# MoseleyBioinformaticsLab/ICIKendallTau

Measured on AMD Instinct MI355X. Metric: column-pairs/s (+ full-matrix wall time) at 10k feat x 1k samp, higher is better.
Workload: dtype int32 rank/popcount counting + f64 epilogue

## Files before the change

### icikendalltau_amd/csrc/icikt_capi.cpp

```cpp
#include <hip/hip_runtime.h>

#include <algorithm>
#include <chrono>
#include <cstdio>
#include <cstring>
#include <functional>
#include <new>
#include <string>
#include <vector>

#include "icikt.h"
#include "icikt_device.h"
#include "icikt_host.h"

using icikt::ColStats;
using icikt::PairRaw;
using icikt::PrepView;

static_assert(ICIKT_CNT_FIELDS == icikt::ICIKT_CNT_FIELDS_, "counts record layout");
static_assert(ICIKT_PERSPECTIVE_LOCAL == icikt::ICIKT_PERSPECTIVE_LOCAL_, "perspective code");

namespace {

int flush_timer(icikt_ctx* c, int k) {
// ... 578 lines not shown
  pv.sort_keys = c->sort_keys.p; pv.sort_idx = c->sort_idx.p;
  pv.tgroups = c->tgroups.p;
  pv.tprog = c->tprog.p;
  pv.srow = c->srow.p;
  pv.smask = c->smask.p;
  if (pv.wide) {
    pv.order32 = c->wide32.p;
    pv.q32 = pv.order32 + S * (size_t)pv.n_pad;
    pv.lo32 = pv.q32 + S * (size_t)pv.n_pad;
    pv.hi32 = pv.lo32 + S * (size_t)pv.n_pad;
    pv.k0_bits = c->k0_bits.p;
  }
  c->pv = pv;
  c->alloc_cols = (int64_t)S;
  return ICIKT_SUCCESS;
}

int mask_alloc(icikt_ctx* c, int64_t n_feat, int64_t n_samp) {
  c->prepared = false;
  c->raw_valid = false;
  PrepView pv{};
  pv.n = (int)n_feat;
  pv.n_pad = std::max(64, (int)((n_feat + 63) / 64 * 64));
  pv.W = (int)((n_feat + 63) / 64);
  pv.Wp = pv.W + 1;
  pv.n_samp = (int)n_samp;
  pv.mstride = pv.Wp;
  HIPCHK(c, c->meta.reserve((size_t)std::max<int64_t>(n_samp, 1) * (size_t)pv.mstride));
  pv.meta = c->meta.p;
  c->pv = pv;
  return ICIKT_SUCCESS;
}

int prepare_launch(icikt_ctx* c, const double* dX, int64_t ld, int64_t col_begin, int64_t col_end, hipStream_t stream) {
  const PrepView& pv = c->pv;
  if (!stream) stream = c->stream;
  c->raw_valid = false;
  c->tied_state = -1;
  c->ntg_hint = -1;
  c->group_hint = 0;
  if (col_end > col_begin)
    HIPCHK(c, hipMemsetAsync(c->meta.p + (size_t)col_begin * pv.mstride, 0,
                             (size_t)(col_end - col_begin) * pv.mstride * sizeof(unsigned long long), stream));
  if (pv.n > 0) {
    const int64_t chunk = std::max(1, c->sort_chunk);
    for (int64_t c0 = col_begin; c0 < col_end; c0 += chunk) {
      const int nc = (int)std::min<int64_t>(chunk, col_end - c0);
      const int small_shape = (c->k0_shape == 1 || (c->k0_shape < 0 && c->k0_small)) ? 1 : 0;
      HIPCHK(c, icikt::launch_k0(pv, dX, ld, (int)c0, nc, c->k0_mask, c->k0_keep, small_shape, stream));
    }
  }
  return ICIKT_SUCCESS;
}

}
}

using icikt::host::prepare_alloc;
using icikt::host::prepare_launch;

static int prepare_impl(icikt_ctx* c, const double* dX, int64_t n_feat, int64_t n_samp, int64_t ld,
                        int64_t col_begin, int64_t col_end, int64_t alloc_cols, uint32_t flags) {
  if (!c) return ICIKT_E_INVALID;
  int rc = check_shape(c, "prepare", n_feat, n_samp, ld);
  if (rc) return rc;
  if (n_samp > 0 && n_feat > 0 && !dX) return fail(c, ICIKT_E_INVALID, "prepare: null matrix");
  rc = check_col_range(c, n_samp, col_begin, col_end, alloc_cols, n_feat);
  if (rc) return rc;
  rc = use_device(c);
  if (rc) return rc;
  rc = prepare_alloc(c, n_feat, n_samp, alloc_cols, col_end - col_begin);
  if (rc) return rc;
  rc = timer_begin(c, ICIKT_K_PREPARE, flags);
  if (rc) return rc;
  rc = prepare_launch(c, dX, ld, col_begin, col_end);
  if (rc) return rc;
  rc = timer_end(c, ICIKT_K_PREPARE, flags);
  if (rc) return rc;
  c->prepared = true;
  return ICIKT_SUCCESS;
}

// ... 836 lines not shown
extern "C" {

int icikt_debug_set_plan(icikt_ctx* c, const char* spec) {
  if (!c) return ICIKT_E_INVALID;
  icikt_ctx::PlanOverride ov;
  int pipe = -1, k0 = -1;
  std::string sp = spec ? spec : "";
  size_t pos = 0;
  while (pos < sp.size()) {
    size_t end = sp.find(',', pos);
    if (end == std::string::npos) end = sp.size();
    const std::string item = sp.substr(pos, end - pos);
    pos = end + 1;
    if (item.empty()) continue;
    const size_t eq = item.find('=');
    if (eq == std::string::npos) return fail(c, ICIKT_E_INVALID, "debug_set_plan: expected key=value, got '" + item + "'");
    const std::string key = item.substr(0, eq), val = item.substr(eq + 1);
    if (val.empty()) continue;
    if (key == "np") ov.np = atoi(val.c_str());
    else if (key == "pend") ov.pend = (val[0] == 'g') ? 1 : 0;
    else if (key == "wpb") ov.wpb = atoi(val.c_str());
    else if (key == "half") ov.half = (val[0] == '1') ? 1 : 0;
    else if (key == "hyb") ov.hyb = (val[0] == '1') ? 1 : 0;
    else if (key == "tgmax") { ov.has_tgmax = true; ov.tgmax = atoi(val.c_str()); }
    else if (key == "list") ov.list = atoi(val.c_str());
    else if (key == "solo") ov.solo = atoi(val.c_str());
    else if (key == "split") ov.split = atoi(val.c_str());
    else if (key == "merge") ov.merge = atoi(val.c_str());
    else if (key == "waves") ov.waves = atoi(val.c_str());
    else if (key == "verbose") ov.verbose = (val[0] == '1');
    else if (key == "gridmult") ov.grid_mult = atoi(val.c_str());
    else if (key == "gridcap") ov.grid_cap = atoi(val.c_str());
    else if (key == "pipe") pipe = (val[0] == '1') ? 1 : 0;
    else if (key == "k0") k0 = (val[0] == '1') ? 1 : 0;
    else if (key == "tkblock") ov.tkblock = atoll(val.c_str());
    else if (key == "medlds") {
      ov.medlds = atoi(val.c_str());
      if (ov.medlds < 0 || ov.medlds > icikt::MEDIAN_STAGE_MAX)
        return fail(c, ICIKT_E_INVALID, "debug_set_plan: medlds must be in 0 .. 4096 keys");
    }
    else if (key == "qbatch") {
      ov.qbatch = atoi(val.c_str());
      if (ov.qbatch < 1 || ov.qbatch > icikt::QUANT_BATCH_MAX)
        return fail(c, ICIKT_E_INVALID, "debug_set_plan: qbatch must be in 1 .. 32 targets");
    }
    else if (key == "padjtile") {
      ov.padjtile = atoll(val.c_str());
      if (ov.padjtile < 1 || ov.padjtile > (1ll << 30))
        return fail(c, ICIKT_E_INVALID, "debug_set_plan: padjtile must be in 1 .. 2^30 keys");
    }
    else if (key == "anoperms") {
      ov.anoperms = atoll(val.c_str());
      if (ov.anoperms < 1 || ov.anoperms > icikt::ANO_PERMS_MAX)
        return fail(c, ICIKT_E_INVALID, "debug_set_plan: anoperms must be in 1 .. 2^20 labellings");
    }
    else if (key == "anostrip") {
      ov.anostrip = atoi(val.c_str());
      if (ov.anostrip < icikt::ANO_STRIP_MIN || ov.anostrip > icikt::ANO_STRIP_MAX)
        return fail(c, ICIKT_E_INVALID, "debug_set_plan: anostrip must be in 1 .. 4096 columns");
    }
    else if (key == "hcgrid") {
      ov.hcgrid = atoi(val.c_str());
      if (ov.hcgrid < 1 || ov.hcgrid > icikt::HCLUST_GRID_MAX)
        return fail(c, ICIKT_E_INVALID, "debug_set_plan: hcgrid must be in 1 .. 256 workgroups");
    }
    else return fail(c, ICIKT_E_INVALID, "debug_set_plan: unknown key '" + key + "'");
  }
// ... 76 lines not shown
```

### icikendalltau_amd/csrc/icikt_device.h

```cpp
#ifndef ICIKT_DEVICE_H
#define ICIKT_DEVICE_H

#include <hip/hip_runtime.h>
#include <stdint.h>

namespace icikt {

constexpr int ICIKT_PERSPECTIVE_LOCAL_ = 0;
constexpr int ICIKT_CNT_FIELDS_ = 11;

struct ColStats {
  int32_t nna;
  int32_t ngroups;
  int32_t tfill;
  int32_t maxgroup;
  uint32_t s0, s1, s2;
  uint32_t ntg;
  long long e0, e1, e2;
  double fill;
  int32_t nexcl;
  int32_t flags;
};
constexpr int COL_ODD_TIE = 1;
__host__ __device__ inline uint32_t col_stream_cost(const ColStats& st) { return (uint32_t)st.flags >> 8; }
// ... 74 lines not shown
  uint32_t* hi32;
  unsigned long long* k0_bits;
};

constexpr int K1_TL_BYTES = 1024 + 256 + 256 + 512 + 64;

__host__ __device__ inline int k1_half_pre(int half_items) { return 32 * (half_items > 8 ? 16 : 8) * 2; }

constexpr int ICIKT_HALF_ITEMS_MAX = 15;
__host__ __device__ inline int k1_half_items(int Wp) {
  const int hi = (Wp + 31) >> 5;
  return (hi >= 8 && (hi & 1) == 0) ? hi + 1 : hi;
}

__host__ __device__ inline int k1_lds_stride(int Wp, int half_items) {
  if (half_items > 0) return 32 * half_items;
  return (Wp + 7) & ~7;
}

constexpr int K1_OPT_HALF = 1;
constexpr int K1_OPT_ROW_ONLY = 2;
constexpr int K1_OPT_HALF_LAYOUT = 4;
constexpr int K1_OPT_NO_SOLO = 8;
constexpr int K1_OPT_SEG_SHIFT = 4;
constexpr int K1_OPT_LIST_SHIFT = 8, K1_OPT_LIST_MASK = 0x3FF;
constexpr int K1_OPT_CNT_SHIFT = 18;
__host__ __device__ constexpr int k1_opt_segments(int opts) { return 1 << ((opts >> K1_OPT_SEG_SHIFT) & 3); }
__host__ __device__ constexpr int k1_opt_tg_list(int opts) { return (opts >> K1_OPT_LIST_SHIFT) & K1_OPT_LIST_MASK; }
__host__ __device__ constexpr int k1_opt_cnt_cap(int opts) { return opts >> K1_OPT_CNT_SHIFT; }
__host__ __device__ constexpr int k1_opt_pack_segments(int split) { return (split == 4 ? 2 : split == 2 ? 1 : 0) << K1_OPT_SEG_SHIFT; }
__host__ __device__ constexpr int k1_opt_pack_tg_list(int tg_list) { return tg_list << K1_OPT_LIST_SHIFT; }
__host__ __device__ constexpr int k1_opt_pack_cnt_cap(int entries) { return entries << K1_OPT_CNT_SHIFT; }

hipError_t launch_k0(const PrepView& pv, const double* dX, int64_t ld, int col_begin, int ncols, const MaskSpec* ms,
                     uint8_t* keep, int small_shape, hipStream_t s);
hipError_t launch_out_stats(const PrepView& pv, const double* out4, const int32_t* reasons, int64_t n_pairs,
                            const int64_t* n_good, unsigned long long* red, hipStream_t s);
hipError_t launch_assemble(const PrepView& pv, const double* out4, const int32_t* pi, const int32_t* pj, int64_t n_pairs,
                           const int64_t* n_good, const unsigned long long* red, int scale_max, int diag_good,
                           double* out5, hipStream_t s);
hipError_t launch_out_stats_accum(const PrepView& pv, const double* out4, const int32_t* reasons, int64_t n_pairs,
                                  unsigned long long* red, hipStream_t s);
struct TopkLists {
  unsigned long long* key;
  int32_t* partner;
  double* vals;
  int32_t* count;
  int32_t* cur;
  int k;
};
hipError_t launch_topk_merge(const TopkLists& L, const double* out4, int S, int row_a, int row_b, hipStream_t s);
hipError_t launch_topk_finish(const TopkLists& L, const unsigned long long* red, int S, int scale_max, int32_t* idx,
                              double* out5k, int32_t* n_valid, hipStream_t s);
struct EdgeRule {
  double min_raw, max_pvalue, min_completeness;
  int absolute;
};
struct EdgeOut {
  int32_t *ei, *ej;
  double *cor, *raw, *pvalue, *taumax, *completeness;
  long long cap;
};
long long edge_tiles(long long n_pairs);
constexpr int EDGE_TILE_WORDS = 16;
hipError_t launch_edge_block(const EdgeRule& R, const double* out4, long long n_pairs, long long first, int S,
                             unsigned long long* ballots, uint32_t* counts, unsigned long long* bases,
                             unsigned long long* total, unsigned long long* degree, const EdgeOut& E, hipStream_t s);
hipError_t launch_edge_finish(const EdgeOut& E, long long n, const unsigned long long* red, int scale_max, hipStream_t s);
// ... 171 lines not shown
```

### icikendalltau_amd/csrc/icikt_prepass.hip

```cpp
#include <hip/hip_runtime.h>
#include <stdint.h>
#include <stdlib.h>

#include <algorithm>
#include <type_traits>

#include "icikt_device.h"
#include "icikt_wave.h"

namespace icikt {

constexpr int K0_THREADS = 1024;
constexpr int K0_THREADS_SMALL = 256;
#ifndef ICIKT_K0_MIN_WAVES
#define ICIKT_K0_MIN_WAVES 4
#endif
#ifndef ICIKT_K0_WAVES_SMALL
#define ICIKT_K0_WAVES_SMALL 5
#endif
constexpr int K0_UB = 8;
#ifdef ICIKT_K0_NO_NETWORK
constexpr bool K0_NETWORK = false;
#else
constexpr bool K0_NETWORK = true;
#endif
constexpr int K0_TILE = 4096;

__device__ __forceinline__ unsigned long long sortable_key(double v) {
  if (v == 0.0) v = 0.0;
  long long b = __double_as_longlong(v);
  unsigned long long u = (unsigned long long)b;
  return (b < 0) ? ~u : (u | 0x8000000000000000ull);
}

template <bool FAST>
__device__ __forceinline__ bool kv_gt(unsigned long long ka, uint32_t ia, unsigned long long kb, uint32_t ib) {
  if constexpr (FAST) return ka > kb;
  return (ka > kb) || (ka == kb && ia > ib);
}
template <bool FAST, int E>
__device__ __forceinline__ void k0_reg_stages(unsigned long long (&ek)[E], uint32_t (&ei)[E], int k, int jmax,
                                              int gi, int tid) {
  const uint32_t lane = (uint32_t)tid & 63u;
  const bool upw = (gi & k) == 0;
#define ICIKT_K0_XSTAGE(LX)                                                                              \
  if (jmax >= E * (LX)) {                                                                                \
    const bool want_gt = (((tid & (LX)) == 0) == upw);  \
    _Pragma("unroll") for (int r = 0; r < E; ++r) {                                                      \
      const uint32_t klo = lane_xor<(LX)>((uint32_t)ek[r], lane), khi = lane_xor<(LX)>((uint32_t)(ek[r] >> 32), lane); \
      const uint32_t oi = FAST ? 0u : lane_xor<(LX)>(ei[r], lane);                                       \
      const unsigned long long ok = (unsigned long long)klo | ((unsigned long long)khi << 32);           \
      if (kv_gt<FAST>(ek[r], ei[r], ok, oi) == want_gt) { ek[r] = ok; ei[r] = oi; }                      \
    }                                                                                                    \
  }
  ICIKT_K0_XSTAGE(32) ICIKT_K0_XSTAGE(16) ICIKT_K0_XSTAGE(8) ICIKT_K0_XSTAGE(4) ICIKT_K0_XSTAGE(2) ICIKT_K0_XSTAGE(1)
#undef ICIKT_K0_XSTAGE
#pragma unroll
  for (int j = E / 2; j >= 1; j >>= 1) {
    if (jmax >= j) {
#pragma unroll
      for (int a = 0; a < E; ++a) {
        if ((a & j) == 0) {
          const int b = a | j;
          const bool up = ((gi + a) & k) == 0;
          if (kv_gt<FAST>(ek[a], ei[a], ek[b], ei[b]) == up) {
// ... 227 lines not shown

template <bool WIDE, int NT, int E>
__device__ __forceinline__ void k0_prepare_body(const PrepView& pv, const double* __restrict__ X, int64_t ld, int col_begin,
                                                const MaskSpec& ms, uint8_t* __restrict__ keep) {
  static_assert((NT == K0_THREADS || NT == K0_THREADS_SMALL) && (E == 4 || E == 8 || E == 16), "pre-pass shapes");
  constexpr int TILE = NT * E;
  constexpr int NW = NT / 64;
  __shared__ long long sh_ll[K0_THREADS];
  __shared__ int sh_i[K0_THREADS];
  __shared__ unsigned long long sh_bits_lds[1024];
  __shared__ unsigned long long sh_st_lds[1028];
  unsigned long long* const sh_bits = WIDE ? pv.k0_bits + (size_t)blockIdx.x * 2 * (size_t)(pv.Wp + 1) : sh_bits_lds;
  unsigned long long* const sh_st = WIDE ? sh_bits + (pv.Wp + 1) : sh_st_lds;
  __shared__ unsigned long long sh_sort[TILE + TILE / 2];
  __shared__ uint16_t sh_bigpre[1024];
  unsigned long long* sh_tk = sh_sort;
  uint32_t* sh_ti = reinterpret_cast<uint32_t*>(sh_sort + TILE);
  uint32_t* rec_s = reinterpret_cast<uint32_t*>(sh_sort);
  const bool stage_hg = !WIDE && pv.n_pad <= 3 * TILE;
  const bool stage_rec = stage_hg && 2 * pv.n_pad <= 3 * TILE;
  uint32_t* hg_s = stage_rec ? rec_s + pv.n_pad : rec_s;
  bool want_gi = pv.tp_stride > 0;

  const int c = col_begin + blockIdx.x;
  const int tid = threadIdx.x;
  const int lane = tid & 63;
  const int n = pv.n;
  const int W = pv.W;
  const int npow2 = pv.npow2;
  const double* col = X + (int64_t)c * ld;
  unsigned long long* keys = pv.sort_keys + (int64_t)blockIdx.x * npow2;
  uint32_t* idx = pv.sort_idx + (int64_t)blockIdx.x * npow2;
  unsigned long long* mask = pv.col_mask(c);
  unsigned long long* fmask = pv.col_fillmask(c);
  unsigned long long* gflag = pv.col_gflag(c);
  uint16_t* order = WIDE ? nullptr : pv.order + (int64_t)c * pv.n_ord;
  uint32_t* rec = WIDE ? nullptr : pv.rec + ((int64_t)(c >> 1) * pv.rec_rows) * 2 + (c & 1);
  uint16_t* hirow = WIDE ? nullptr : pv.hirow + ((int64_t)(c >> 1) * pv.rec_rows) * 2 + (c & 1);
  uint16_t* girow = WIDE ? nullptr : pv.girow + ((int64_t)(c >> 1) * pv.rec_rows) * 2 + (c & 1);
  if (!WIDE && tid == 0) {
    rec[2 * pv.n_pad] = (uint32_t)pv.n_pad; hirow[2 * pv.n_pad] = 0; girow[2 * pv.n_pad] = GIROW_NONE;
  }
  uint32_t* tgl = WIDE ? nullptr : pv.tgroups + (int64_t)c * pv.tg_stride;
  uint32_t* order32 = WIDE ? pv.order32 + (int64_t)c * pv.n_pad : nullptr;
  uint32_t* q32 = WIDE ? pv.q32 + (int64_t)c * pv.n_pad : nullptr;
  uint32_t* lo32 = WIDE ? pv.lo32 + (int64_t)c * pv.n_pad : nullptr;
  uint32_t* hi32 = WIDE ? pv.hi32 + (int64_t)c * pv.n_pad : nullptr;

  double tmin = __longlong_as_double(0x7FF0000000000000ll);
  int nna = 0, nexcl = 0;
  uint8_t* keep_c = keep ? keep + (int64_t)c * n : nullptr;
  for (int base0 = 0; base0 < pv.n_pad; base0 += NT * K0_UB) {
    double vv[K0_UB];
#pragma unroll
    for (int u = 0; u < K0_UB; ++u) {
      const int i = base0 + u * NT + tid;
      vv[u] = (i < n) ? col[i] : 0.0;
    }
#pragma unroll
    for (int u = 0; u < K0_UB; ++u) {
      if (base0 + u * NT < pv.n_pad) {
        const int i = base0 + u * NT + tid;
        const double v = vv[u];
        const bool excl = (i < n) && mask_excluded(ms, v);
        const bool isna = (i < n) && (excl || v != v);
        nexcl += excl ? 1 : 0;
        if (keep_c && i < n) keep_c[i] = excl ? 0 : 1;
        const unsigned long long b = __ballot(isna);
        if (lane == 0 && (i >> 6) < W) {
          mask[i >> 6] = b;
          if (!WIDE) sh_bits_lds[i >> 6] = b;
        }
        if (i < n && !isna) tmin = (v < tmin) ? v : tmin;
        nna += isna ? 1 : 0;
      }
    }
  }
  if (tid == 0) { mask[W] = 0ull; }
  {
    tmin = wave_reduce(tmin, [](double a, double b) { return (b < a) ? b : a; });
    nna = wave_reduce(nna, [](int a, int b) { return a + b; });
    nexcl = wave_reduce(nexcl, [](int a, int b) { return a + b; });
    double* sh_d = reinterpret_cast<double*>(sh_st_lds);
    if (lane == 0) { sh_d[tid >> 6] = tmin; sh_i[tid >> 6] = nna; sh_i[NW + (tid >> 6)] = nexcl; }
    __syncthreads();
    tmin = sh_d[0]; nna = sh_i[0]; nexcl = sh_i[NW];
#pragma unroll
    for (int w = 1; w < NW; ++w) {
      const double b = sh_d[w];
      tmin = (b < tmin) ? b : tmin;
      nna += sh_i[w];
      nexcl += sh_i[NW + w];
    }
    __syncthreads();
  }
  const double fill = tmin - 0.1;

  auto sort_plan = [&](int x, int& np2, int& nreal, int& m, int& sub_lo) -> int {
    np2 = npow2; nreal = x; m = 0; sub_lo = 0;
    if (npow2 < TILE) return np2;
    const int F = x / TILE, r = x - F * TILE;
    const int rp2 = (r <= 64 * E) ? 64 * E : (1 << (32 - __builtin_clz((uint32_t)(r - 1))));
    if (rp2 == TILE) np2 = 1 << (32 - __builtin_clz((uint32_t)(x - 1)));
    else if (F == 0) { np2 = 0; nreal = 0; m = rp2; }
    else if ((F & (F - 1)) == 0 && r > 0) { np2 = nreal = F * TILE; m = rp2; sub_lo = K0_NETWORK ? TILE - m : 0; }
    else np2 = 1 << (32 - __builtin_clz((uint32_t)(x - 1)));
    return np2 + m;
  };
  int cna = 0;
  if constexpr (!WIDE) {
    int a0, a1, a2, a3;
    if (nna > 0 && fill < tmin && sort_plan(n - nna, a0, a1, a2, a3) < sort_plan(n, a0, a1, a2, a3)) {
      cna = nna;
      int pbase = 0;
      for (int wb = 0; wb < W; wb += NT) {
        const int wi = wb + tid;
        const int cnt = (wi < W) ? (int)__popcll(sh_bits_lds[wi]) : 0;
        const int incl = (int)wave_incl_scan((uint32_t)cnt);
        if (lane == 63) sh_i[tid >> 6] = incl;
        __syncthreads();
        int wbase = pbase, btot = 0;
        for (int w = 0; w < NW; ++w) {
          const int t = sh_i[w];
          if (w < (tid >> 6)) wbase += t;
          btot += t;
        }
        if (wi < W) sh_bigpre[wi] = (uint16_t)(wbase + incl - cnt);
        pbase += btot;
        __syncthreads();
// ... 214 lines not shown
      for (int u = 0; u < K0_UB; ++u) {
        const int k = base0 + u * NT + tid;
        vv[u] = (k < n) ? col[rowv[u]] : 0.0;
        vp[u] = (lane == 0 && k > 0 && k < n) ? col[rowp[u]] : 0.0;
      }
#pragma unroll
      for (int u = 0; u < K0_UB; ++u) {
        if (base0 + u * NT <= ((n >> 6) << 6)) {
          const int k = base0 + u * NT + tid;
          unsigned long long fk = 0ull;
          if (k < n) {
            double v = vv[u];
            if (v != v || mask_excluded(ms, v)) v = fill;
            fk = sortable_key(v);
            if (k >= cna) idx[k] = rowv[u];
          }
          unsigned long long prev = __shfl_up(fk, 1, 64);
          if (lane == 0 && k > 0 && k < n) {
            double v = vp[u];
            if (v != v || mask_excluded(ms, v)) v = fill;
            prev = sortable_key(v);
          }
          const bool st = (k <= n) && (k == 0 || k == n || prev != fk);
          inv |= (k > 0 && k < n && prev > fk) ? 1 : 0;
          const unsigned long long b = __ballot(st);
          if (lane == 0 && (k >> 6) <= (n >> 6)) sh_st[k >> 6] = b;
        }
      }
    }
    if (__syncthreads_or(inv) && K0_NETWORK) sort_pass(std::false_type{});
    else starts_done = true;
  }

  if (!starts_done) {
    for (int base = 0; base <= ((n >> 6) << 6); base += NT) {
      const int k = base + tid;
      const bool st = (k <= n) && (k == 0 || k == n || keys[k - 1] != keys[k]);
      const unsigned long long b = __ballot(st);
      if (lane == 0 && (k >> 6) <= (n >> 6)) sh_st[k >> 6] = b;
    }
  }
  unsigned long long* sh_big = reinterpret_cast<unsigned long long*>(sh_ll);
  for (int w = tid; w < (WIDE ? pv.Wp : 1024); w += NT) sh_bits[w] = 0ull;
  if (WIDE) {
    for (int k = n + tid; k < pv.n_pad; k += NT) order32[k] = 0u;
  } else {
    for (int k = n + tid; k < pv.n_ord; k += NT) order[k] = 0;
    if (pv.order_w) { for (int k = n + tid; k < pv.n_ord; k += NT) pv.order_w[(int64_t)c * pv.n_ord + k] = 0u; }
  }
  __syncthreads();
  auto is_start = [&](int k) -> bool { return (sh_st[k >> 6] >> (k & 63)) & 1ull; };
  auto prev_start = [&](int k) -> int {
    int w = k >> 6;
    unsigned long long m = sh_st[w] & (~0ull >> (63 - (k & 63)));
    while (m == 0ull) m = sh_st[--w];
    return (w << 6) + 63 - (int)__builtin_clzll(m);
  };
  auto next_start = [&](int k) -> int {
    const int q = k + 1;
    int w = q >> 6;
    unsigned long long m = sh_st[w] & (~0ull << (q & 63));
    while (m == 0ull) m = sh_st[++w];
    return (w << 6) + (int)__builtin_ctzll(m);
  };

  if (!WIDE) {
    const int nw = (n + 63) >> 6;
    int gbase = 0;
    for (int wb = 0; wb < nw; wb += NT) {
      const int wi = wb + tid;
      unsigned long long bg = 0ull;
      if (wi < nw) {
        const unsigned long long st = sh_st[wi];
        bg = st & ~((st >> 1) | (sh_st[wi + 1] << 63));
        const int last = n - 1 - wi * 64;
        if (last < 63) bg &= (2ull << last) - 1ull;
        sh_big[wi] = bg;
      }
      const int cnt = (int)__popcll(bg);
      const int incl = (int)wave_incl_scan((uint32_t)cnt);
      if (lane == 63) sh_i[tid >> 6] = incl;
      __syncthreads();
      int wbase = gbase, btot = 0;
      for (int w = 0; w < NW; ++w) {
        const int t = sh_i[w];
        if (w < (tid >> 6)) wbase += t;
        btot += t;
      }
      if (wi < nw) sh_bigpre[wi] = (uint16_t)(wbase + incl - cnt);
      gbase += btot;
      __syncthreads();
    }
    want_gi = want_gi || gbase > K1_CNT_MIN_GROUPS;
  }

  int ngroups = 0, maxgroup = 0, tfill = 0, ntg_local = 0, oddtie = 0;
  uint32_t s0 = 0, s1 = 0, s2 = 0;
  long long e0 = 0, e1 = 0, e2 = 0;
  for (int base0 = 0; base0 < n; base0 += NT * K0_UB) {
    uint32_t rows[K0_UB];
#pragma unroll
    for (int u = 0; u < K0_UB; ++u) {
      const int k = base0 + u * NT + tid;
      rows[u] = (k < n) ? idx[k] : 0u;
    }
#pragma unroll
    for (int u = 0; u < K0_UB; ++u) {
    if (base0 + u * NT >= n) break;
    const int k = base0 + u * NT + tid;
    if (k < n) {
      const int lo = prev_start(k), hi = next_start(k) - 1;
      const uint32_t row = rows[u];
      if (WIDE) {
        hi32[row] = (uint32_t)hi; q32[row] = (uint32_t)k; lo32[row] = (uint32_t)lo;
        order32[n - 1 - k] = row;
      } else {
      const uint32_t gi = (want_gi && hi > lo) ? ((uint32_t)sh_bigpre[lo >> 6] + (uint32_t)__popcll(sh_big[lo >> 6] & ((1ull << (lo & 63)) - 1ull)))
                                               : (uint32_t)GIROW_NONE;
      if (stage_hg) hg_s[row] = (uint32_t)hi | (gi << 16);
      else { hirow[2 * row] = (uint16_t)hi; if (want_gi) girow[2 * row] = (uint16_t)gi; }
      if (stage_rec) rec_s[row] = (uint32_t)k | ((uint32_t)lo << 16);
      else rec[2 * row] = (uint32_t)k | ((uint32_t)lo << 16);
      order[n - 1 - k] = (uint16_t)row;
      if (pv.order_w) pv.order_w[(int64_t)c * pv.n_ord + (n - 1 - k)] = row;
      }
      if (lo == 0 && nna > 0) atomicOr(&sh_bits[row >> 6], 1ull << (row & 63));
      if (lo == k) {
        const int t = hi - lo + 1;
        ++ngroups;
        if (!WIDE) maxgroup = (int)max((uint32_t)maxgroup, ((uint32_t)t << 16) | (uint32_t)lo);
        if (lo == 0) tfill = t;
        if (t >= 2) {
          ++ntg_local;
          oddtie |= lo & 1;
          const uint32_t ut = (uint32_t)t;
          const uint32_t tt1 = ut * (ut - 1u);
          s0 += tt1;
          s1 += tt1 * (ut - 2u);
          s2 += tt1 * (2u * ut + 5u);
          const long long lt = t;
          e0 += lt * (lt - 1);
          e1 += lt * (lt - 1) * (lt - 2);
          e2 += lt * (lt - 1) * (2 * lt + 5);
        }
      }
    }
    }
  }
  __syncthreads();
  if (stage_rec) {
    for (int r = tid; r < n; r += NT) rec[2 * r] = rec_s[r];
  }
  if (stage_hg) {
    for (int r = tid; r < n; r += NT) {
      const uint32_t hg = hg_s[r];
      hirow[2 * r] = (uint16_t)hg;
      if (want_gi) girow[2 * r] = (uint16_t)(hg >> 16);
    }
  }

  for (int base = 0; base < pv.n_pad; base += NT) {
    const int kp = base + tid;
    bool flag = false;
    if (kp < n) {
      const int k = n - 1 - kp;
      flag = is_start(k + 1);
    }
    const unsigned long long b = __ballot(flag);
    if (lane == 0 && (kp >> 6) < W) gflag[kp >> 6] = b;
  }
  if (tid == 0) { gflag[W] = 0ull; }
  for (int w = tid; w <= W; w += NT) fmask[w] = (w < W) ? sh_bits[w] : 0ull;
  int stream_cost = 2 * ((n + 63) >> 6);
  if (!WIDE && pv.tp_stride > 0) {
    __syncthreads();
    for (int base = 0; base < pv.n_pad; base += NT) {
      const int kp = base + tid;
      const bool flag = (kp < n) && is_start(n - kp);
      const unsigned long long b = __ballot(flag);
      if (lane == 0 && (kp >> 6) < W) sh_bits_lds[kp >> 6] = b;
    }
    if (tid == 0) sh_bits_lds[W] = 0ull;
    __syncthreads();
    uint16_t* Ewin = reinterpret_cast<uint16_t*>(sh_sort);
    uint32_t* crossT = reinterpret_cast<uint32_t*>(Ewin + TPROG_WIN);
    uint16_t* mlist = reinterpret_cast<uint16_t*>(crossT + 2048);
    k0_tie_program(sh_bits_lds, Ewin, mlist, crossT, &sh_i[0], n, W, pv.tprog + (int64_t)c * pv.tp_stride,
                   pv.tprog + (int64_t)c * pv.tp_stride + (pv.tp_stride - 2 * TPROG_MARKS), order,
                   pv.srow + (int64_t)c * pv.sr_steps * 64, pv.smask + (int64_t)c * pv.sr_steps * 32, pv.sr_steps,
                   (uint32_t)pv.n_pad, tid, NT);
    stream_cost = sh_i[3];
    __syncthreads();
  }

  if (!WIDE) {
    const int nw = (n + 63) >> 6;
    for (int wi = tid; wi < nw; wi += NT) {
      int off = (int)sh_bigpre[wi];
      unsigned long long m = sh_big[wi];
      while (m != 0ull) {
        const int k = (wi << 6) + (int)__builtin_ctzll(m);
        m &= m - 1ull;
        tgl[off++] = (uint32_t)k | ((uint32_t)(next_start(k) - 1) << 16);
      }
    }
  }
  const auto add_i = [](int a, int b) { return a + b; };
  const auto add_u = [](uint32_t a, uint32_t b) { return a + b; };
  const auto add_l = [](long long a, long long b) { return a + b; };
  const int ntg_w = wave_reduce(ntg_local, add_i);
  ngroups = wave_reduce(ngroups, add_i);
  maxgroup = (int)wave_reduce((uint32_t)maxgroup, [](uint32_t a, uint32_t b) { return a > b ? a : b; });
  tfill = wave_reduce(tfill, [](int a, int b) { return a > b ? a : b; });
  oddtie = wave_reduce(oddtie, [](int a, int b) { return a | b; });
  s0 = wave_reduce(s0, add_u); s1 = wave_reduce(s1, add_u); s2 = wave_reduce(s2, add_u);
  e0 = wave_reduce(e0, add_l); e1 = wave_reduce(e1, add_l); e2 = wave_reduce(e2, add_l);
  __syncthreads();
  if (lane == 0) {
    int* wi = sh_i + (tid >> 6) * 8;
    wi[0] = ntg_w; wi[1] = ngroups; wi[2] = maxgroup; wi[3] = tfill; wi[4] = oddtie; wi[5] = (int)s0; wi[6] = (int)s1; wi[7] = (int)s2;
    long long* wl = sh_ll + (tid >> 6) * 3;
    wl[0] = e0; wl[1] = e1; wl[2] = e2;
  }
  __syncthreads();
  int ntg = 0;
  if (tid == 0) {
    ngroups = 0; maxgroup = 0; tfill = 0; oddtie = 0; s0 = s1 = s2 = 0u; e0 = e1 = e2 = 0;
    for (int w = 0; w < NW; ++w) {
      const int* wi = sh_i + w * 8;
      ntg += wi[0]; ngroups += wi[1];
      maxgroup = ((uint32_t)wi[2] > (uint32_t)maxgroup) ? wi[2] : maxgroup;
      tfill = max(tfill, wi[3]); oddtie |= wi[4];
      s0 += (uint32_t)wi[5]; s1 += (uint32_t)wi[6]; s2 += (uint32_t)wi[7];
      const long long* wl = sh_ll + w * 3;
      e0 += wl[0]; e1 += wl[1]; e2 += wl[2];
    }
  }

  if (tid == 0) {
    ColStats st;
    st.nna = nna;
    st.ngroups = ngroups;
    st.tfill = (nna > 0) ? tfill : 0;
    st.maxgroup = maxgroup;
    st.s0 = s0; st.s1 = s1; st.s2 = s2; st.ntg = (uint32_t)ntg;
    st.e0 = e0; st.e1 = e1; st.e2 = e2;
    st.fill = fill;
    st.nexcl = nexcl;
    st.flags = (oddtie ? COL_ODD_TIE : 0) | (int32_t)((uint32_t)min(stream_cost, 0xFFFFFF) << 8);
    *pv.col_stats(c) = st;
  }
}

__global__ void __launch_bounds__(K0_THREADS, ICIKT_K0_MIN_WAVES)
k0_prepare_large(PrepView pv, const double* __restrict__ X, int64_t ld, int col_begin, const MaskSpec ms, uint8_t* __restrict__ keep) {
  k0_prepare_body<false, K0_THREADS, 4>(pv, X, ld, col_begin, ms, keep);
}
__global__ void __launch_bounds__(K0_THREADS, ICIKT_K0_MIN_WAVES)
k0_prepare_large8(PrepView pv, const double* __restrict__ X, int64_t ld, int col_begin, const MaskSpec ms, uint8_t* __restrict__ keep) {
  k0_prepare_body<false, K0_THREADS, 8>(pv, X, ld, col_begin, ms, keep);
}
__global__ void __launch_bounds__(K0_THREADS, ICIKT_K0_MIN_WAVES)
k0_prepare_wide(PrepView pv, const double* __restrict__ X, int64_t ld, int col_begin, const MaskSpec ms, uint8_t* __restrict__ keep) {
  k0_prepare_body<true, K0_THREADS, K0_TILE / K0_THREADS>(pv, X, ld, col_begin, ms, keep);
}
__global__ void __launch_bounds__(K0_THREADS, ICIKT_K0_WAVES_SMALL)
k0_prepare_small(PrepView pv, const double* __restrict__ X, int64_t ld, int col_begin, const MaskSpec ms, uint8_t* __restrict__ keep) {
  k0_prepare_body<false, K0_THREADS_SMALL, K0_TILE / K0_THREADS_SMALL>(pv, X, ld, col_begin, ms, keep);
}

constexpr int KX_WAVES = 4;
__global__ void __launch_bounds__(64 * KX_WAVES) k0_expand(PrepView pv, int col_begin, int ncols, int staged) {
  extern __shared__ __attribute__((aligned(16))) unsigned char kx_stage[];
  uint32_t* rec_s = reinterpret_cast<uint32_t*>(kx_stage);
  uint16_t* hi_s = reinterpret_cast<uint16_t*>(kx_stage + (size_t)pv.n_pad * 4);
  uint16_t* gi_s = reinterpret_cast<uint16_t*>(kx_stage + (size_t)pv.n_pad * 6);
  __shared__ __attribute__((aligned(8))) int prevs[1032];
  __shared__ int nexts[1032];
  __shared__ int msuf[1032];
  __shared__ uint32_t kx_cross[32 * 64];
  __shared__ uint16_t kx_E[TPROG_WIN];
  __shared__ uint16_t kx_list[2 * TPROG_LIST];
  __shared__ int kx_cnt[24];
  const int wave = (int)(threadIdx.x >> 6);
  const int lane = (int)(threadIdx.x & 63);
  const int c = col_begin + (int)blockIdx.x;
  const int n = pv.n, W = pv.W, Wp = pv.Wp;
  const unsigned long long* gf = pv.col_gflag(c);
  const uint16_t* ord = pv.order + (int64_t)c * pv.n_ord;
  uint32_t* rec = pv.rec + ((int64_t)(c >> 1) * pv.rec_rows) * 2 + (c & 1);
  uint16_t* hirow = pv.hirow + ((int64_t)(c >> 1) * pv.rec_rows) * 2 + (c & 1);
  uint16_t* girow = pv.girow + ((int64_t)(c >> 1) * pv.rec_rows) * 2 + (c & 1);
  uint32_t* tgl = pv.tgroups + (int64_t)c * pv.tg_stride;
  if (threadIdx.x == 0) {
    rec[2 * pv.n_pad] = (uint32_t)pv.n_pad; hirow[2 * pv.n_pad] = 0; girow[2 * pv.n_pad] = GIROW_NONE;
  }
  if (pv.order_w) {
    uint32_t* ow = pv.order_w + (int64_t)c * pv.n_ord;
    for (int k = (int)threadIdx.x; k < pv.n_ord; k += (int)blockDim.x) ow[k] = (uint32_t)ord[k];
  }

// ... 73 lines not shown
      girow[2 * r] = gi_s[r];
    }
  }
  if (pv.tp_stride > 0) {
    __syncthreads();
    unsigned long long* gfl = reinterpret_cast<unsigned long long*>(prevs);
    for (int w = (int)threadIdx.x; w <= W; w += 64 * KX_WAVES) gfl[w] = gf[w];
    __syncthreads();
    k0_tie_program(gfl, kx_E, kx_list, kx_cross, kx_cnt, n, W, pv.tprog + (int64_t)c * pv.tp_stride,
                   pv.tprog + (int64_t)c * pv.tp_stride + (pv.tp_stride - 2 * TPROG_MARKS), ord,
                   pv.srow + (int64_t)c * pv.sr_steps * 64, pv.smask + (int64_t)c * pv.sr_steps * 32, pv.sr_steps,
                   (uint32_t)pv.n_pad, (int)threadIdx.x, 64 * KX_WAVES);
  }
}

constexpr int KM_WORDS = 64;
__global__ void __launch_bounds__(256)
k0_mask(PrepView pv, const double* __restrict__ X, int64_t ld, int col_begin) {
  const int c = col_begin + (int)blockIdx.x;
  const double* col = X + (int64_t)c * ld;
  unsigned long long* mask = pv.col_mask(c);
  const int lane = (int)(threadIdx.x & 63u), wave = (int)(threadIdx.x >> 6);
  const int w0 = (int)blockIdx.y * KM_WORDS;
  for (int w = w0 + wave; w < min(w0 + KM_WORDS, pv.W); w += 4) {
    const int i = w * 64 + lane;
    const double v = (i < pv.n) ? col[i] : 0.0;
    const unsigned long long b = __ballot(v != v);
    if (lane == 0) mask[w] = b;
  }
  if (blockIdx.y == 0 && threadIdx.x == 0) mask[pv.W] = 0ull;
}

hipError_t launch_k0(const PrepView& pv, const double* dX, int64_t ld, int col_begin, int ncols, const MaskSpec* msp,
                     uint8_t* keep, int small_shape, hipStream_t s) {
  (void)hipGetLastError();
  MaskSpec ms{};
  if (msp) ms = *msp;
  if (pv.wide)
    hipLaunchKernelGGL(k0_prepare_wide, dim3(ncols), dim3(K0_THREADS), 0, s, pv, dX, ld, col_begin, ms, keep);
  else if (small_shape)
    hipLaunchKernelGGL(k0_prepare_small, dim3(ncols), dim3(K0_THREADS_SMALL), 0, s, pv, dX, ld, col_begin, ms, keep);
  else if (pv.npow2 >= 2 * K0_TILE)
    hipLaunchKernelGGL(k0_prepare_large8, dim3(ncols), dim3(K0_THREADS), 0, s, pv, dX, ld, col_begin, ms, keep);
  else
    hipLaunchKernelGGL(k0_prepare_large, dim3(ncols), dim3(K0_THREADS), 0, s, pv, dX, ld, col_begin, ms, keep);
  return hipGetLastError();
}

hipError_t launch_k0_expand(const PrepView& pv, int col_begin, int ncols, hipStream_t s) {
  if (ncols <= 0 || pv.n <= 0) return hipSuccess;
  (void)hipGetLastError();
  const int staged = (pv.n_pad <= 12288) ? 1 : 0;
  const size_t lds = staged ? (size_t)pv.n_pad * 8 : 0;
  if (staged) {
    hipError_t e = hipFuncSetAttribute(reinterpret_cast<const void*>(k0_expand), hipFuncAttributeMaxDynamicSharedMemorySize, (int)lds);
    if (e != hipSuccess) return e;
  }
  hipLaunchKernelGGL(k0_expand, dim3(ncols), dim3(64 * KX_WAVES), lds, s, pv, col_begin, ncols, staged);
  return hipGetLastError();
}

hipError_t launch_k0_mask(const PrepView& pv, const double* dX, int64_t ld, int col_begin, int ncols, hipStream_t s) {
  if (ncols <= 0) return hipSuccess;
  (void)hipGetLastError();
  const unsigned slabs = (unsigned)std::max(1, (pv.W + KM_WORDS - 1) / KM_WORDS);
  hipLaunchKernelGGL(k0_mask, dim3((unsigned)ncols, slabs), dim3(256), 0, s, pv, dX, ld, col_begin);
  return hipGetLastError();
}

}
```

### icikendalltau_amd/csrc/icikt_wave.h

```cpp
#ifndef ICIKT_WAVE_H
#define ICIKT_WAVE_H

#include <hip/hip_runtime.h>
#include <stdint.h>

namespace icikt {

__device__ __forceinline__ uint32_t lane_id() { return threadIdx.x & 63u; }

__device__ __forceinline__ uint32_t dpp_wave_shr1(uint32_t old, uint32_t src) {
  return (uint32_t)__builtin_amdgcn_update_dpp((int)old, (int)src, 0x138 , 0xf, 0xf, false);
}

__device__ __forceinline__ uint32_t wave_incl_scan(uint32_t v) {
  v += (uint32_t)__builtin_amdgcn_update_dpp(0, (int)v, 0x111, 0xf, 0xf, false);
  v += (uint32_t)__builtin_amdgcn_update_dpp(0, (int)v, 0x112, 0xf, 0xf, false);
  v += (uint32_t)__builtin_amdgcn_update_dpp(0, (int)v, 0x114, 0xf, 0xf, false);
  v += (uint32_t)__builtin_amdgcn_update_dpp(0, (int)v, 0x118, 0xf, 0xf, false);
  v += (uint32_t)__builtin_amdgcn_update_dpp(0, (int)v, 0x142 , 0xa, 0xf, false);
  v += (uint32_t)__builtin_amdgcn_update_dpp(0, (int)v, 0x143 , 0xc, 0xf, false);
  return v;
}

template <int X>
// ... 41 lines not shown

__device__ __forceinline__ uint32_t gload_u32(const uint32_t* base, uint32_t idx) {
  return *reinterpret_cast<const uint32_t*>(reinterpret_cast<const char*>(base) + (size_t)(idx << 2));
}
__device__ __forceinline__ uint32_t gload_u16(const uint16_t* base, uint32_t idx) {
  return *reinterpret_cast<const uint16_t*>(reinterpret_cast<const char*>(base) + (size_t)(idx << 1));
}

__device__ __forceinline__ uint2 gload_rec2(const uint32_t* blk, uint32_t row) {
  return *reinterpret_cast<const uint2*>(reinterpret_cast<const char*>(blk) + (size_t)(row << 3));
}

__device__ __forceinline__ void seen_insert(unsigned long long* bits, uint32_t pos) {
  atomicOr(reinterpret_cast<uint32_t*>(bits) + (pos >> 5), 1u << (pos & 31u));
}

__device__ __forceinline__ uint32_t bcnt_acc(uint32_t x, uint32_t acc) {
  uint32_t r;
  asm("v_bcnt_u32_b32 %0, %1, %2" : "=v"(r) : "v"(x), "v"(acc));
  return r;
}
__device__ __forceinline__ uint32_t pack16(uint32_t hi, uint32_t lo) {
  uint32_t r;
  asm("v_lshl_or_b32 %0, %1, 16, %2" : "=v"(r) : "v"(hi), "v"(lo));
  return r;
}
__device__ __forceinline__ uint32_t bcnt64_acc(unsigned long long x, uint32_t acc) {
  return bcnt_acc((uint32_t)(x >> 32), bcnt_acc((uint32_t)x, acc));
}
__device__ __forceinline__ unsigned long long low_mask64(uint32_t bits ) {
  return (1ull << bits) - 1ull;
}

template <typename T, typename Op>
__device__ __forceinline__ T wave_reduce(T v, Op op) {
#pragma unroll
  for (int o = 32; o > 0; o >>= 1) v = op(v, __shfl_xor(v, o, 64));
  return v;
}
template <int J>
__device__ __forceinline__ uint32_t lane_xor(uint32_t v, uint32_t lane) {
  if (J == 1) return (uint32_t)__builtin_amdgcn_update_dpp(0, (int)v, 0xB1 , 0xf, 0xf, false);
  if (J == 2) return (uint32_t)__builtin_amdgcn_update_dpp(0, (int)v, 0x4E , 0xf, 0xf, false);
  if (J == 4) {
    const uint32_t up = (uint32_t)__builtin_amdgcn_update_dpp(0, (int)v, 0x104 , 0xf, 0xf, false);
    const uint32_t dn = (uint32_t)__builtin_amdgcn_update_dpp(0, (int)v, 0x114 , 0xf, 0xf, false);
    return (lane & 4u) ? dn : up;
  }
  if (J == 8) return (uint32_t)__builtin_amdgcn_update_dpp(0, (int)v, 0x128 , 0xf, 0xf, false);
  if (J == 16) {
    const auto r = __builtin_amdgcn_permlane16_swap(v, v, false, false);
    return (lane & 16u) ? r[0] : r[1];
  }
  const auto r = __builtin_amdgcn_permlane32_swap(v, v, false, false);
  return (lane & 32u) ? r[0] : r[1];
}

}
#endif
```

Before: 54.49 million.

## Trim K0 prepass register pressure and add two-per-CU kernel shape

Moves the per-column output pointer setup to after the sort phase to shorten live ranges, and drops the separate 32-bit tie sums by deriving them from the 64-bit sums. It replaces the serial cross-wave min/sum loop with a wave reduction and makes reduced values wave-uniform via readfirstlane. wave_reduce now uses swizzle/permlane xor instead of __shfl_xor. It also adds an optional K0 variant with higher launch-bounds occupancy, selectable by a debug key but not used by default.

```diff
diff --git a/icikendalltau_amd/csrc/icikt_capi.cpp b/icikendalltau_amd/csrc/icikt_capi.cpp
--- a/icikendalltau_amd/csrc/icikt_capi.cpp
+++ b/icikendalltau_amd/csrc/icikt_capi.cpp
@@ -634,6 +634,13 @@
   return ICIKT_SUCCESS;
 }
 
+static int k0_pick_shape(const icikt_ctx* c, const PrepView& pv) {
+  if (pv.wide) return icikt::K0_SHAPE_LARGE;
+  if (c->k0_shape == 1 || (c->k0_shape < 0 && c->k0_small)) return icikt::K0_SHAPE_SMALL;
+  if (c->k0_shape == 2) return icikt::K0_SHAPE_TWO;
+  return icikt::K0_SHAPE_LARGE;
+}
+
 int prepare_launch(icikt_ctx* c, const double* dX, int64_t ld, int64_t col_begin, int64_t col_end, hipStream_t stream) {
   const PrepView& pv = c->pv;
   if (!stream) stream = c->stream;
@@ -648,8 +655,12 @@
     const int64_t chunk = std::max(1, c->sort_chunk);
     for (int64_t c0 = col_begin; c0 < col_end; c0 += chunk) {
       const int nc = (int)std::min<int64_t>(chunk, col_end - c0);
-      const int small_shape = (c->k0_shape == 1 || (c->k0_shape < 0 && c->k0_small)) ? 1 : 0;
-      HIPCHK(c, icikt::launch_k0(pv, dX, ld, (int)c0, nc, c->k0_mask, c->k0_keep, small_shape, stream));
+      const int shape = k0_pick_shape(c, pv);
+      if (c->plan_ov.verbose)
+        fprintf(stderr, "[icikt] K0 plan: %d columns x %d rows on %d CUs, shape=%s%s\n", nc, pv.n, c->prop.multiProcessorCount,
+                pv.wide ? "wide" : shape == icikt::K0_SHAPE_TWO ? "two_per_cu" : shape == icikt::K0_SHAPE_SMALL ? "small" : "large",
+                c->k0_shape >= 0 ? " (forced)" : "");
+      HIPCHK(c, icikt::launch_k0(pv, dX, ld, (int)c0, nc, c->k0_mask, c->k0_keep, shape, stream));
     }
   }
   return ICIKT_SUCCESS;
@@ -1552,7 +1563,7 @@
     else if (key == "gridmult") ov.grid_mult = atoi(val.c_str());
     else if (key == "gridcap") ov.grid_cap = atoi(val.c_str());
     else if (key == "pipe") pipe = (val[0] == '1') ? 1 : 0;
-    else if (key == "k0") k0 = (val[0] == '1') ? 1 : 0;
+    else if (key == "k0") k0 = (val[0] == '2') ? 2 : (val[0] == '1') ? 1 : 0;
     else if (key == "tkblock") ov.tkblock = atoll(val.c_str());
     else if (key == "medlds") {
       ov.medlds = atoi(val.c_str());
diff --git a/icikendalltau_amd/csrc/icikt_device.h b/icikendalltau_amd/csrc/icikt_device.h
--- a/icikendalltau_amd/csrc/icikt_device.h
+++ b/icikendalltau_amd/csrc/icikt_device.h
@@ -130,8 +130,9 @@
 __host__ __device__ constexpr int k1_opt_pack_tg_list(int tg_list) { return tg_list << K1_OPT_LIST_SHIFT; }
 __host__ __device__ constexpr int k1_opt_pack_cnt_cap(int entries) { return entries << K1_OPT_CNT_SHIFT; }
 
+constexpr int K0_SHAPE_LARGE = 0, K0_SHAPE_SMALL = 1, K0_SHAPE_TWO = 2;
 hipError_t launch_k0(const PrepView& pv, const double* dX, int64_t ld, int col_begin, int ncols, const MaskSpec* ms,
-                     uint8_t* keep, int small_shape, hipStream_t s);
+                     uint8_t* keep, int shape, hipStream_t s);
 hipError_t launch_out_stats(const PrepView& pv, const double* out4, const int32_t* reasons, int64_t n_pairs,
                             const int64_t* n_good, unsigned long long* red, hipStream_t s);
 hipError_t launch_assemble(const PrepView& pv, const double* out4, const int32_t* pi, const int32_t* pj, int64_t n_pairs,
diff --git a/icikendalltau_amd/csrc/icikt_prepass.hip b/icikendalltau_amd/csrc/icikt_prepass.hip
--- a/icikendalltau_amd/csrc/icikt_prepass.hip
+++ b/icikendalltau_amd/csrc/icikt_prepass.hip
@@ -31,6 +31,12 @@
   long long b = __double_as_longlong(v);
   unsigned long long u = (unsigned long long)b;
   return (b < 0) ? ~u : (u | 0x8000000000000000ull);
+}
+
+__device__ __forceinline__ double uniform_f64(double v) {
+  const long long b = __double_as_longlong(v);
+  const uint32_t hi = (uint32_t)__builtin_amdgcn_readfirstlane((int)(b >> 32)), lo = (uint32_t)__builtin_amdgcn_readfirstlane((int)b);
+  return __longlong_as_double((long long)(((unsigned long long)hi << 32) | lo));
 }
 
 template <bool FAST>
@@ -324,21 +330,6 @@
   unsigned long long* keys = pv.sort_keys + (int64_t)blockIdx.x * npow2;
   uint32_t* idx = pv.sort_idx + (int64_t)blockIdx.x * npow2;
   unsigned long long* mask = pv.col_mask(c);
-  unsigned long long* fmask = pv.col_fillmask(c);
-  unsigned long long* gflag = pv.col_gflag(c);
-  uint16_t* order = WIDE ? nullptr : pv.order + (int64_t)c * pv.n_ord;
-  uint32_t* rec = WIDE ? nullptr : pv.rec + ((int64_t)(c >> 1) * pv.rec_rows) * 2 + (c & 1);
-  uint16_t* hirow = WIDE ? nullptr : pv.hirow + ((int64_t)(c >> 1) * pv.rec_rows) * 2 + (c & 1);
-  uint16_t* girow = WIDE ? nullptr : pv.girow + ((int64_t)(c >> 1) * pv.rec_rows) * 2 + (c & 1);
-  if (!WIDE && tid == 0) {
-    rec[2 * pv.n_pad] = (uint32_t)pv.n_pad; hirow[2 * pv.n_pad] = 0; girow[2 * pv.n_pad] = GIROW_NONE;
-  }
-  uint32_t* tgl = WIDE ? nullptr : pv.tgroups + (int64_t)c * pv.tg_stride;
-  uint32_t* order32 = WIDE ? pv.order32 + (int64_t)c * pv.n_pad : nullptr;
-  uint32_t* q32 = WIDE ? pv.q32 + (int64_t)c * pv.n_pad : nullptr;
-  uint32_t* lo32 = WIDE ? pv.lo32 + (int64_t)c * pv.n_pad : nullptr;
-  uint32_t* hi32 = WIDE ? pv.hi32 + (int64_t)c * pv.n_pad : nullptr;
-
   double tmin = __longlong_as_double(0x7FF0000000000000ll);
   int nna = 0, nexcl = 0;
   uint8_t* keep_c = keep ? keep + (int64_t)c * n : nullptr;
@@ -376,17 +367,17 @@
     double* sh_d = reinterpret_cast<double*>(sh_st_lds);
     if (lane == 0) { sh_d[tid >> 6] = tmin; sh_i[tid >> 6] = nna; sh_i[NW + (tid >> 6)] = nexcl; }
     __syncthreads();
-    tmin = sh_d[0]; nna = sh_i[0]; nexcl = sh_i[NW];
-#pragma unroll
-    for (int w = 1; w < NW; ++w) {
-      const double b = sh_d[w];
-      tmin = (b < tmin) ? b : tmin;
-      nna += sh_i[w];
-      nexcl += sh_i[NW + w];
-    }
-    __syncthreads();
-  }
-  const double fill = tmin - 0.1;
+    {
+      const double t = sh_d[lane & (NW - 1)];
+      const int a = (lane < NW) ? sh_i[lane] : 0, b = (lane < NW) ? sh_i[NW + lane] : 0;
+      tmin = wave_reduce(t, [](double x, double y) { return (y < x) ? y : x; });
+      nna = __builtin_amdgcn_readfirstlane(wave_reduce(a, [](int x, int y) { return x + y; }));
+      nexcl = __builtin_amdgcn_readfirstlane(wave_reduce(b, [](int x, int y) { return x + y; }));
+      tmin = uniform_f64(tmin);
+    }
+    __syncthreads();
+  }
+  const double fill = uniform_f64(tmin - 0.1);
 
   auto sort_plan = [&](int x, int& np2, int& nreal, int& m, int& sub_lo) -> int {
     np2 = npow2; nreal = x; m = 0; sub_lo = 0;
@@ -667,6 +658,21 @@
     else starts_done = true;
   }
 
+  unsigned long long* fmask = pv.col_fillmask(c);
+  unsigned long long* gflag = pv.col_gflag(c);
+  uint16_t* order = WIDE ? nullptr : pv.order + (int64_t)c * pv.n_ord;
+  uint32_t* rec = WIDE ? nullptr : pv.rec + ((int64_t)(c >> 1) * pv.rec_rows) * 2 + (c & 1);
+  uint16_t* hirow = WIDE ? nullptr : pv.hirow + ((int64_t)(c >> 1) * pv.rec_rows) * 2 + (c & 1);
+  uint16_t* girow = WIDE ? nullptr : pv.girow + ((int64_t)(c >> 1) * pv.rec_rows) * 2 + (c & 1);
+  if (!WIDE && tid == 0) {
+    rec[2 * pv.n_pad] = (uint32_t)pv.n_pad; hirow[2 * pv.n_pad] = 0; girow[2 * pv.n_pad] = GIROW_NONE;
+  }
+  uint32_t* tgl = WIDE ? nullptr : pv.tgroups + (int64_t)c * pv.tg_stride;
+  uint32_t* order32 = WIDE ? pv.order32 + (int64_t)c * pv.n_pad : nullptr;
+  uint32_t* q32 = WIDE ? pv.q32 + (int64_t)c * pv.n_pad : nullptr;
+  uint32_t* lo32 = WIDE ? pv.lo32 + (int64_t)c * pv.n_pad : nullptr;
+  uint32_t* hi32 = WIDE ? pv.hi32 + (int64_t)c * pv.n_pad : nullptr;
+
   if (!starts_done) {
     for (int base = 0; base <= ((n >> 6) << 6); base += NT) {
       const int k = base + tid;
@@ -730,7 +736,6 @@
   }
 
   int ngroups = 0, maxgroup = 0, tfill = 0, ntg_local = 0, oddtie = 0;
-  uint32_t s0 = 0, s1 = 0, s2 = 0;
   long long e0 = 0, e1 = 0, e2 = 0;
   for (int base0 = 0; base0 < n; base0 += NT * K0_UB) {
     uint32_t rows[K0_UB];
@@ -768,11 +773,6 @@
         if (t >= 2) {
           ++ntg_local;
           oddtie |= lo & 1;
-          const uint32_t ut = (uint32_t)t;
-          const uint32_t tt1 = ut * (ut - 1u);
-          s0 += tt1;
-          s1 += tt1 * (ut - 2u);
-          s2 += tt1 * (2u * ut + 5u);
           const long long lt = t;
           e0 += lt * (lt - 1);
           e1 += lt * (lt - 1) * (lt - 2);
@@ -782,6 +782,16 @@
     }
     }
   }
+  const auto add_i = [](int a, int b) { return a + b; };
+  const auto add_l = [](long long a, long long b) { return a + b; };
+  const int ntg_w = __builtin_amdgcn_readfirstlane(wave_reduce(ntg_local, add_i));
+  ngroups = __builtin_amdgcn_readfirstlane(wave_reduce(ngroups, add_i));
+  maxgroup = __builtin_amdgcn_readfirstlane((int)wave_reduce((uint32_t)maxgroup, [](uint32_t a, uint32_t b) { return a > b ? a : b; }));
+  tfill = __builtin_amdgcn_readfirstlane(wave_reduce(tfill, [](int a, int b) { return a > b ? a : b; }));
+  oddtie = __builtin_amdgcn_readfirstlane(wave_reduce(oddtie, [](int a, int b) { return a | b; }));
+  e0 = (long long)uniform_u64((unsigned long long)wave_reduce(e0, add_l));
+  e1 = (long long)uniform_u64((unsigned long long)wave_reduce(e1, add_l));
+  e2 = (long long)uniform_u64((unsigned long long)wave_reduce(e2, add_l));
   __syncthreads();
   if (stage_rec) {
     for (int r = tid; r < n; r += NT) rec[2 * r] = rec_s[r];
@@ -840,33 +850,22 @@
       }
     }
   }
-  const auto add_i = [](int a, int b) { return a + b; };
-  const auto add_u = [](uint32_t a, uint32_t b) { return a + b; };
-  const auto add_l = [](long long a, long long b) { return a + b; };
-  const int ntg_w = wave_reduce(ntg_local, add_i);
-  ngroups = wave_reduce(ngroups, add_i);
-  maxgroup = (int)wave_reduce((uint32_t)maxgroup, [](uint32_t a, uint32_t b) { return a > b ? a : b; });
-  tfill = wave_reduce(tfill, [](int a, int b) { return a > b ? a : b; });
-  oddtie = wave_reduce(oddtie, [](int a, int b) { return a | b; });
-  s0 = wave_reduce(s0, add_u); s1 = wave_reduce(s1, add_u); s2 = wave_reduce(s2, add_u);
-  e0 = wave_reduce(e0, add_l); e1 = wave_reduce(e1, add_l); e2 = wave_reduce(e2, add_l);
   __syncthreads();
   if (lane == 0) {
     int* wi = sh_i + (tid >> 6) * 8;
-    wi[0] = ntg_w; wi[1] = ngroups; wi[2] = maxgroup; wi[3] = tfill; wi[4] = oddtie; wi[5] = (int)s0; wi[6] = (int)s1; wi[7] = (int)s2;
+    wi[0] = ntg_w; wi[1] = ngroups; wi[2] = maxgroup; wi[3] = tfill; wi[4] = oddtie;
     long long* wl = sh_ll + (tid >> 6) * 3;
     wl[0] = e0; wl[1] = e1; wl[2] = e2;
   }
   __syncthreads();
   int ntg = 0;
   if (tid == 0) {
-    ngroups = 0; maxgroup = 0; tfill = 0; oddtie = 0; s0 = s1 = s2 = 0u; e0 = e1 = e2 = 0;
+    ngroups = 0; maxgroup = 0; tfill = 0; oddtie = 0; e0 = e1 = e2 = 0;
     for (int w = 0; w < NW; ++w) {
       const int* wi = sh_i + w * 8;
       ntg += wi[0]; ngroups += wi[1];
       maxgroup = ((uint32_t)wi[2] > (uint32_t)maxgroup) ? wi[2] : maxgroup;
       tfill = max(tfill, wi[3]); oddtie |= wi[4];
-      s0 += (uint32_t)wi[5]; s1 += (uint32_t)wi[6]; s2 += (uint32_t)wi[7];
       const long long* wl = sh_ll + w * 3;
       e0 += wl[0]; e1 += wl[1]; e2 += wl[2];
     }
@@ -878,7 +877,7 @@
     st.ngroups = ngroups;
     st.tfill = (nna > 0) ? tfill : 0;
     st.maxgroup = maxgroup;
-    st.s0 = s0; st.s1 = s1; st.s2 = s2; st.ntg = (uint32_t)ntg;
+    st.s0 = (uint32_t)e0; st.s1 = (uint32_t)e1; st.s2 = (uint32_t)e2; st.ntg = (uint32_t)ntg;
     st.e0 = e0; st.e1 = e1; st.e2 = e2;
     st.fill = fill;
     st.nexcl = nexcl;
@@ -902,6 +901,11 @@
 __global__ void __launch_bounds__(K0_THREADS, ICIKT_K0_WAVES_SMALL)
 k0_prepare_small(PrepView pv, const double* __restrict__ X, int64_t ld, int col_begin, const MaskSpec ms, uint8_t* __restrict__ keep) {
   k0_prepare_body<false, K0_THREADS_SMALL, K0_TILE / K0_THREADS_SMALL>(pv, X, ld, col_begin, ms, keep);
+}
+constexpr int K0_WAVES_TWO = 8;
+__global__ void __launch_bounds__(K0_THREADS, K0_WAVES_TWO)
+k0_prepare_two(PrepView pv, const double* __restrict__ X, int64_t ld, int col_begin, const MaskSpec ms, uint8_t* __restrict__ keep) {
+  k0_prepare_body<false, K0_THREADS, K0_TILE / K0_THREADS>(pv, X, ld, col_begin, ms, keep);
 }
 
 constexpr int KX_WAVES = 4;
@@ -1041,13 +1045,15 @@
 }
 
 hipError_t launch_k0(const PrepView& pv, const double* dX, int64_t ld, int col_begin, int ncols, const MaskSpec* msp,
-                     uint8_t* keep, int small_shape, hipStream_t s) {
+                     uint8_t* keep, int shape, hipStream_t s) {
   (void)hipGetLastError();
   MaskSpec ms{};
   if (msp) ms = *msp;
   if (pv.wide)
     hipLaunchKernelGGL(k0_prepare_wide, dim3(ncols), dim3(K0_THREADS), 0, s, pv, dX, ld, col_begin, ms, keep);
-  else if (small_shape)
+  else if (shape == K0_SHAPE_TWO)
+    hipLaunchKernelGGL(k0_prepare_two, dim3(ncols), dim3(K0_THREADS), 0, s, pv, dX, ld, col_begin, ms, keep);
+  else if (shape == K0_SHAPE_SMALL)
     hipLaunchKernelGGL(k0_prepare_small, dim3(ncols), dim3(K0_THREADS_SMALL), 0, s, pv, dX, ld, col_begin, ms, keep);
   else if (pv.npow2 >= 2 * K0_TILE)
     hipLaunchKernelGGL(k0_prepare_large8, dim3(ncols), dim3(K0_THREADS), 0, s, pv, dX, ld, col_begin, ms, keep);
diff --git a/icikendalltau_amd/csrc/icikt_wave.h b/icikendalltau_amd/csrc/icikt_wave.h
--- a/icikendalltau_amd/csrc/icikt_wave.h
+++ b/icikendalltau_amd/csrc/icikt_wave.h
@@ -97,10 +97,27 @@
   return (1ull << bits) - 1ull;
 }
 
+template <int X, typename T>
+__device__ __forceinline__ T wave_xor_get(T v) {
+  static_assert(sizeof(T) == 4 || sizeof(T) == 8, "wave_xor_get: 32- or 64-bit values");
+  if constexpr (sizeof(T) == 4) {
+    const uint32_t u = __builtin_bit_cast(uint32_t, v);
+    return __builtin_bit_cast(T, (X == 32) ? xor32(u) : swz_xor<(X & 31)>(u));
+  } else {
+    const unsigned long long u = __builtin_bit_cast(unsigned long long, v);
+    const uint32_t lo = (uint32_t)u, hi = (uint32_t)(u >> 32);
+    const uint32_t l2 = (X == 32) ? xor32(lo) : swz_xor<(X & 31)>(lo), h2 = (X == 32) ? xor32(hi) : swz_xor<(X & 31)>(hi);
+    return __builtin_bit_cast(T, (unsigned long long)l2 | ((unsigned long long)h2 << 32));
+  }
+}
 template <typename T, typename Op>
 __device__ __forceinline__ T wave_reduce(T v, Op op) {
-#pragma unroll
-  for (int o = 32; o > 0; o >>= 1) v = op(v, __shfl_xor(v, o, 64));
+  v = op(v, wave_xor_get<32>(v));
+  v = op(v, wave_xor_get<16>(v));
+  v = op(v, wave_xor_get<8>(v));
+  v = op(v, wave_xor_get<4>(v));
+  v = op(v, wave_xor_get<2>(v));
+  v = op(v, wave_xor_get<1>(v));
   return v;
 }
 template <int J>
```

Result: no change. 54.58 million (median of 3 runs) (+0.2%).
